# asharakeh/pod_compare

Measured on AMD Instinct MI355X. Metric: images/sec (BayesOD+MC-dropout, 1280x720), higher is better.
Workload: dtype f32 (convolutions: every fp32 product from 2-way f16 splits of the power-of-two-scaled fp32 operands, 3 partial products, fp32 accumulate; closer to fp64 than the fp32 MFMA: profiles/r05_f16_split_numerics.txt)

## Files before the change

### pod_compare_amd/csrc/k12_wino_conv_split.hip

```cpp
#include "pod_wino.h"

namespace pod {

typedef uint32_t vu32x4 __attribute__((ext_vector_type(4)));
constexpr int WINO_US_BYTES = 24 * 2 * 2 * 64 * 16;
constexpr int WINO_U_TOP = 14, WINO_V_TOP = 9;
constexpr int WINO_WAIT_VM24 = 0x4078;
constexpr int WINO_TAIL_NO_LOAD = 1, WINO_TAIL_NO_PARK = 2, WINO_TAIL_LAST = 4;

__global__ void __launch_bounds__(256) k_wino_filter_amax(const float* __restrict__ w, float* __restrict__ amax, int32_t K, int32_t C, int32_t Kpad) {
    const int64_t t = (int64_t)blockIdx.x * blockDim.x + threadIdx.x;
    float m = 0.0f;
    if (t < (int64_t)Kpad * C) {
        float u[4][6];
        wino_filter_values(w, (int)(t / C), (int)(t % C), K, C, u);
#pragma unroll
        for (int i = 0; i < 24; ++i) m = fmaxf(m, fabsf(u[i / 6][i % 6]));
    }
    wino_publish_amax1(amax, m);
}
__global__ void __launch_bounds__(256) k_wino_filter_split(const float* __restrict__ w, uint16_t* __restrict__ Us, const float* __restrict__ amax,
                                                           int32_t K, int32_t C, int32_t Kpad) {
    const int64_t t = (int64_t)blockIdx.x * blockDim.x + threadIdx.x;
    if (t >= (int64_t)Kpad * C) return;
    const int k = (int)(t / C), c = (int)(t % C);
    float u[4][6];
    wino_filter_values(w, k, c, K, C, u);
    const float sc = wino_pow2_scale(*amax, WINO_U_TOP);
    const int nchunk = C / 16, ks = k >> 6, kb = (k >> 5) & 1, j32 = k & 31, ch = c >> 4, hh = (c >> 3) & 1, e = c & 7;
    uint16_t* dst = Us + (((int64_t)ks * nchunk + ch) * (int64_t)WINO_US_BYTES) / 2 + (hh * 32 + j32) * 8 + e;
#pragma unroll
    for (int a = 0; a < 4; ++a)
#pragma unroll
        for (int p = 0; p < 6; ++p) {
            const float x = u[a][p] * sc;
            const _Float16 h0 = (_Float16)x;
            const _Float16 h1 = (_Float16)(x - (float)h0);
            uint16_t* d = dst + (((a * 6 + p) * 2 + kb) * 2) * 512;
            d[0] = __builtin_bit_cast(uint16_t, h0);
            d[512] = __builtin_bit_cast(uint16_t, h1);
        }
}

__global__ void __launch_bounds__(256, 1) k_wino_conv3x3_split(const WinoParams P) {
    extern __shared__ __attribute__((aligned(16))) float lds[];
    const int tid = threadIdx.x, lane = tid & 63, wave = tid >> 6;
    int ks, tb;
    wino_schedule(P.KS, P.n_blocks, ks, tb);
    if (tb >= P.n_blocks) return;
    uint32_t need[2] = {~0u, ~0u};
    if (P.live) {
        if (tb >= P.live[0]) return;
        const int32_t* const ent = P.live + POD_SPARSE_LIVE_HEAD + (int64_t)POD_SPARSE_LIVE_STRIDE * tb;
        tb = ent[0];
        need[0] = (uint32_t)ent[1 + (tid >> 5)];
        need[1] = (uint32_t)ent[9 + (tid >> 5 < 3 ? tid >> 5 : 2)];
    }
    WINO_STAMP(0);
    WINO_STAMP_WALL(12);
    uint32_t slot_e[12];
    int mini_pidx[3], dmini[3], doff[12];
    WINO_FILL_SLOTS(slot_e, mini_pidx, tid);
    const int nchunk_all = P.C >> 4;
    const int nchunk = P.c_split ? P.c_split : nchunk_all;
    const int chunk0 = (int)blockIdx.y * nchunk;
    const int i32 = lane & 31, h = lane >> 5;
    const int a = __builtin_amdgcn_readfirstlane(wave);
    const int set = (tb >= P.sets.first[1] ? 1 : 0) + (tb >= P.sets.first[2] ? 1 : 0) + (tb >= P.sets.first[3] ? 1 : 0);
    const float* const set_U = P.sets.U[set];
    const float* const set_in = P.sets.in[set];
    float* const set_out = P.sets.out[set];
    const float* const set_bias = P.sets.bias[set];
    const float in_amax_slot = wino_load_amax(P.sets.in_amax[set]);
    const float u_amax = *reinterpret_cast<const float*>(reinterpret_cast<const char*>(set_U) + (int64_t)P.KS * (P.C >> 4) * WINO_US_BYTES);
    float* const set_out_amax = P.sets.out_amax[set];
    const uint64_t set_offset = P.sets.offset[set];
    const int set_replicas = P.sets.replicas[set], set_k_planes = P.sets.k_planes[set];
    const auto u_rsrc = __builtin_amdgcn_make_buffer_rsrc(const_cast<char*>(reinterpret_cast<const char*>(set_U) + ((int64_t)ks * nchunk_all + chunk0) * WINO_US_BYTES), 0,
                                                          nchunk * WINO_US_BYTES, 0x00020000);
    const int u_off = (a * 6 * 4 * 64 + h * 32 + i32) * 16;
    constexpr int WINO_U_LEAD = 3;
    vu32x4 uP[6][4];
    auto filter_piece = [&](int q16, int p, vu32x4(&u)[4], int i) {
        u[i] = __builtin_bit_cast(vu32x4, __builtin_amdgcn_raw_buffer_load_b128(u_rsrc, u_off, q16 * WINO_US_BYTES + (p * 4 + i) * 1024, 0));
    };
#pragma unroll
    for (int pp = 0; pp < WINO_U_LEAD; ++pp)
#pragma unroll
        for (int i = 0; i < 4; ++i) filter_piece(0, pp, uP[pp], i);
    const WinoBlock B = wino_block(P.blocks[tb]);
    int row0, row1;
    float sgn;
    wino_rows(a, row0, row1, sgn);
    const int ty = i32 >> 2, tx = i32 & 3;
    const uint32_t lds_base = (uint32_t)(uintptr_t)(__attribute__((address_space(3))) float*)lds;
    uint32_t areg[2][2][2][2];
    uint32_t amini[2];
#pragma unroll
    for (int rs = 0; rs < 2; ++rs) {
        const int py = 2 * ty + (rs ? row1 : row0);
        const int p0 = 2 * (((py & 3) + 4 * (py >> 3)) * 18 + 4 * tx) + ((py >> 2) & 1);
#pragma unroll
        for (int cl = 0; cl < 2; ++cl) {
            const int rot = ((tx + cl) & 3) + 4 * ((py >> 1) & 1);
#pragma unroll
            for (int c16 = 0; c16 < 2; ++c16)
#pragma unroll
                for (int hf = 0; hf < 2; ++hf) areg[rs][cl][c16][hf] = lds_base + p0 * 128 + ((4 * c16 + 2 * h + hf + rot) & 7) * 16;
        }
    }
#pragma unroll
    for (int rs = 0; rs < 2; ++rs) amini[rs] = lds_base + 2 * WINO_SB_FLOATS * 4 + h * 12288 + ((2 * ty + (rs ? row1 : row0)) * 21 + tx) * 32;
    const auto r_rsrc = __builtin_amdgcn_make_buffer_rsrc(const_cast<float*>(set_in + B.base_px * P.in_stride + chunk0 * 16), 0,
                                                          B.n_img * B.HWi * P.in_stride * 4 - chunk0 * 64, 0x00020000);
    int* const pix_tab = wino_pixel_table(lds);
    WINO_FILL_PIXEL_TABLE(pix_tab, B, need, tid);
    wino_mini_offsets(&P, pix_tab, mini_pidx, dmini, lane);
    auto main_offsets = [&]() {
#pragma unroll
        for (int i = 0; i < 12; ++i) doff[i] = pix_tab[slot_e[i] & 0xFFFF];
#pragma unroll
        for (int i = 0; i < 12; ++i) doff[i] = wino_byte_offset(&P, doff[i], 4 * (((lane & 7) - (int)(slot_e[i] >> 16)) & 7));
    };

    f32x4 stg[6];
    const uint32_t stg_addr = lds_base + a * 12288 + lane * 16;
    auto stage_load = [&](int k, int sc, int i) {
        stg[k] = __builtin_bit_cast(f32x4, __builtin_amdgcn_raw_buffer_load_b128(r_rsrc, doff[i], sc * 128, 0));
    };
    auto stage_write = [&](int par, int k, int i) {
        *reinterpret_cast<__attribute__((address_space(3))) f32x4*>((uintptr_t)(stg_addr + par * (WINO_SB_FLOATS * 4) + i * 1024)) = stg[k];
    };

    f32x16 acc[12];
    f32x4 x[12];
    vu32x4 Vb[6][2];
    float tN[6][4], vN[2][6][4];
    if (POD_WINO_ELIM) {
#pragma unroll
    for (int i = 0; i < 12; ++i) Vb[i / 2][i % 2] = vu32x4{0x3c003c00u + i, 0x3c003c00u, 0x3c003c00u, 0x3c003c00u + lane};
#pragma unroll
    for (int i = 0; i < 12; ++i) x[i] = f32x4{1e-3f, 2e-3f, 3e-3f, 4e-3f} * (float)(lane + i);
#pragma unroll
    for (int i = 0; i < 48; ++i) vN[i / 24][(i / 4) % 6][i % 4] = x[i / 4][i % 4];
#pragma unroll
    for (int i = 0; i < 24; ++i) tN[i / 4][i % 4] = x[i / 4][i % 4];
    }
#define WINO_READ(par, c16, hf, i)                                                                                                  \
    asm volatile("ds_read_b128 %0, %1 offset:%2" : "=v"(x[i]) : "v"(areg[(i) / 6][((i) % 6) >> 2][c16][hf]), "i"((par) * WINO_SB_FLOATS * 4 + ((i) % 6) * 256))
#define WINO_READ_MINI(hf, i)                                                                                                        \
    asm volatile("ds_read_b128 %0, %1 offset:%2" : "=v"(x[i]) : "v"(amini[(i) / 6]), "i"((hf) * 16 + ((((i) % 6) & 3) * 5 + (((i) % 6) >> 2)) * 32))
#define WINO_READ12(M, ...)                                                                                                          \
    M(__VA_ARGS__, 0); M(__VA_ARGS__, 1); M(__VA_ARGS__, 2); M(__VA_ARGS__, 3); M(__VA_ARGS__, 4); M(__VA_ARGS__, 5);                \
    M(__VA_ARGS__, 6); M(__VA_ARGS__, 7); M(__VA_ARGS__, 8); M(__VA_ARGS__, 9); M(__VA_ARGS__, 10); M(__VA_ARGS__, 11)
#define WINO_READS_LANDED()                                                                                                           \
    asm volatile("s_waitcnt lgkmcnt(0)" : "+v"(x[0]), "+v"(x[1]), "+v"(x[2]), "+v"(x[3]), "+v"(x[4]), "+v"(x[5]), "+v"(x[6]), "+v"(x[7]), \
                 "+v"(x[8]), "+v"(x[9]), "+v"(x[10]), "+v"(x[11]))
    auto rows_combine = [&](int c0, int c1) __attribute__((always_inline)) {
#pragma unroll
        for (int c = c0; c < c1; ++c) {
#pragma unroll
            for (int e = 0; e < 4; ++e) tN[c][e] = __builtin_fmaf(sgn, x[6 + c][e], x[c][e]);
        }
    };
    float w0s[4], w1s[4], evs[4], ods[4], fs[4], gs[4];
    auto columns_level1 = [&](int e) __attribute__((always_inline)) {
        w0s[e] = __builtin_fmaf(-5.0f, tN[2][e], tN[4][e]);
        w1s[e] = __builtin_fmaf(-5.0f, tN[3][e], tN[5][e]);
        evs[e] = __builtin_fmaf(-4.0f, tN[2][e], tN[4][e]);
        ods[e] = __builtin_fmaf(-4.0f, tN[1][e], tN[3][e]);
        fs[e] = tN[4][e] - tN[2][e];
        gs[e] = tN[3][e] - tN[1][e];
    };
    auto columns_level2 = [&](int hf, int e) __attribute__((always_inline)) {
        vN[hf][0][e] = __builtin_fmaf(4.0f, tN[0][e], w0s[e]);
        vN[hf][5][e] = __builtin_fmaf(4.0f, tN[1][e], w1s[e]);
        vN[hf][1][e] = evs[e] + ods[e];
        vN[hf][2][e] = evs[e] - ods[e];
        vN[hf][3][e] = __builtin_fmaf(2.0f, gs[e], fs[e]);
        vN[hf][4][e] = __builtin_fmaf(-2.0f, gs[e], fs[e]);
    };
    const float sv = __builtin_bit_cast(float, __builtin_amdgcn_readfirstlane(__builtin_bit_cast(int, wino_pow2_scale(wino_reduce_amax(in_amax_slot), WINO_V_TOP))));
    auto split_convert = [&](int p, int term) __attribute__((always_inline)) {
        vu32x4 w;
#pragma unroll
        for (int i = 0; i < 4; ++i) {
            w[i] = term == 0 ? wino_f16_pair_scaled(vN[i >> 1][p][2 * (i & 1)], vN[i >> 1][p][2 * (i & 1) + 1], sv)
                             : wino_f16_pair(vN[i >> 1][p][2 * (i & 1)], vN[i >> 1][p][2 * (i & 1) + 1]);
        }
        Vb[p][term] = w;
    };
    auto split_residual = [&](int p, int i0, int i1) __attribute__((always_inline)) {
#pragma unroll
        for (int i = i0; i < i1; ++i) {
            float& lo = vN[i >> 1][p][2 * (i & 1)];
            float& hi = vN[i >> 1][p][2 * (i & 1) + 1];
            wino_f16_residual_scaled(Vb[p][0][i], lo, hi, sv);
        }
    };
    auto split_position = [&](int p) __attribute__((always_inline)) {
        split_convert(p, 0); split_residual(p, 0, 4); split_convert(p, 1);
    };
    auto make_v = [&](int hf) __attribute__((always_inline)) {
        if (POD_WINO_ELIM & 8) return;
        rows_combine(0, 6);
#pragma unroll
        for (int e = 0; e < 4; ++e) columns_level1(e);
#pragma unroll
        for (int e = 0; e < 4; ++e) columns_level2(hf, e);
    };
    auto split_all = [&]() __attribute__((always_inline)) {
        if (POD_WINO_ELIM & 8) return;
#pragma unroll
        for (int p = 0; p < 6; ++p) split_position(p);
    };

    constexpr int N_UNITS = 58, N_SLOTS = 36;
    auto unit = [&](auto U, auto npar_t, auto n16_t, auto hasA_t) __attribute__((always_inline)) {
        constexpr int u = decltype(U)::value, npar = decltype(npar_t)::value, n16 = decltype(n16_t)::value;
        if constexpr (POD_WINO_ELIM & 8) { if constexpr (u >= 3 && !(u >= 13 && u < 16)) return; }
        if constexpr (u < 3) {
            if constexpr (!(POD_WINO_ELIM & 1)) { WINO_READ(npar, n16, 0, 4 * u); WINO_READ(npar, n16, 0, 4 * u + 1); WINO_READ(npar, n16, 0, 4 * u + 2); WINO_READ(npar, n16, 0, 4 * u + 3); }
        } else if constexpr (u < 7) {
            if constexpr (decltype(hasA_t)::value) {
                constexpr int k = u - 3;
                if constexpr (k == 0) split_convert(5, 0);
                else if constexpr (k == 1) split_residual(5, 0, 2);
                else if constexpr (k == 2) split_residual(5, 2, 4);
                else split_convert(5, 1);
            }
        } else if constexpr (u < 13) {
            if constexpr (u == 7) WINO_READS_LANDED();
            rows_combine(u - 7, u - 6);
        } else if constexpr (u < 16) {
            if constexpr (!(POD_WINO_ELIM & 1)) { WINO_READ(npar, n16, 1, 4 * (u - 13)); WINO_READ(npar, n16, 1, 4 * (u - 13) + 1); WINO_READ(npar, n16, 1, 4 * (u - 13) + 2); WINO_READ(npar, n16, 1, 4 * (u - 13) + 3); }
        } else if constexpr (u < 24) {
            constexpr int k = u - 16;
            if constexpr (k < 4) columns_level1(k);
            else columns_level2(0, k - 4);
        } else if constexpr (u < 30) {
            if constexpr (u == 24) WINO_READS_LANDED();
            rows_combine(u - 24, u - 23);
        } else if constexpr (u < 38) {
            constexpr int k = u - 30;
            if constexpr (k < 4) columns_level1(k);
            else columns_level2(1, k - 4);
        } else {
            constexpr int p = (u - 38) / 4, k = (u - 38) % 4;
            if constexpr (k == 0) split_convert(p, 0);
            else if constexpr (k == 1) split_residual(p, 0, 2);
            else if constexpr (k == 2) split_residual(p, 2, 4);
            else split_convert(p, 1);
        }
    };
    const int last = nchunk - 1, last_s = last >> 1;
    const int sc1 = last_s < 1 ? last_s : 1;
#pragma unroll
    for (int r = 0; r < 3; ++r) wino_mini_piece(r_rsrc, lds, a, 0, r, dmini[r]);
#pragma unroll
    for (int r = 0; r < 3; ++r) wino_mini_piece(r_rsrc, lds, a, 1, r, dmini[r]);
    WINO_STAMP(9);
    main_offsets();
    WINO_STAMP(10);
#pragma unroll
    for (int i = 0; i < 12; ++i) wino_patch_piece(r_rsrc, lds, a, 0, i, doff[i]);
#pragma unroll
    for (int i = 0; i < 6; ++i) wino_patch_piece(r_rsrc, lds + WINO_SB_FLOATS, a, sc1, i, doff[i]);
#pragma unroll
    for (int i = 0; i < 6; ++i) stage_load(i, sc1, 6 + i);
    WINO_STAMP(11);
    __builtin_amdgcn_s_waitcnt(WINO_WAIT_VM24);
    __builtin_amdgcn_s_barrier();
    WINO_STAMP(1);
    WINO_READ12(WINO_READ_MINI, 0);
    WINO_READS_LANDED();
    __builtin_amdgcn_sched_barrier(0);
    make_v(0);
    __builtin_amdgcn_sched_barrier(0);
    WINO_READ12(WINO_READ_MINI, 1);
    WINO_READS_LANDED();
    __builtin_amdgcn_sched_barrier(0);
    make_v(1);
    split_all();
    __builtin_amdgcn_sched_barrier(0);
    WINO_STAMP(2);
    const f32x16 zero16 = {0.f, 0.f, 0.f, 0.f, 0.f, 0.f, 0.f, 0.f, 0.f, 0.f, 0.f, 0.f, 0.f, 0.f, 0.f, 0.f};
    auto chunk = [&](auto mode_t, auto c16_t, auto par_t, auto tail_t, int q) {
        constexpr int mode = decltype(mode_t)::value, c16 = decltype(c16_t)::value, par = decltype(par_t)::value, tail = decltype(tail_t)::value;
        constexpr bool do_load = !(tail & WINO_TAIL_NO_LOAD), do_park = !(tail & WINO_TAIL_NO_PARK), is_last = (tail & WINO_TAIL_LAST) != 0;
        static_assert((tail == 0 || mode == 2) && (!is_last || (!do_load && !do_park)), "tail forms are steady-state chunks; the last one has no stage traffic");
        constexpr int n16 = c16 ^ 1, npar = c16 == 1 ? par ^ 1 : par;
        const int qn = q + 1 <= last ? q + 1 : last;
        const int ls0 = (q >> 1) + 2, ls = ls0 < last_s ? ls0 : last_s;
        wino_static_for([&](auto J) __attribute__((always_inline)) {
            constexpr int j = decltype(J)::value, p = j / 6, m = j % 6, kb = m & 1, prod = m >> 1;
            constexpr int sa = prod == 1 ? 1 : 0;
            constexpr int sb = prod == 0 ? 1 : 0;
            if constexpr (mode == 0 && prod == 0)
                acc[p * 2 + kb] = __builtin_amdgcn_mfma_f32_32x32x16_f16(__builtin_bit_cast(wino_f16x8, uP[p][kb * 2 + sa]), __builtin_bit_cast(wino_f16x8, Vb[p][sb]), zero16, 0, 0, 0);
            else
                acc[p * 2 + kb] = __builtin_amdgcn_mfma_f32_32x32x16_f16(__builtin_bit_cast(wino_f16x8, uP[p][kb * 2 + sa]), __builtin_bit_cast(wino_f16x8, Vb[p][sb]), acc[p * 2 + kb], 0, 0, 0);
            if constexpr (m < 4 && (!is_last || p + WINO_U_LEAD < 6)) { if (!(POD_WINO_ELIM & 2)) filter_piece(p + WINO_U_LEAD >= 6 ? qn : q, (p + WINO_U_LEAD) % 6, uP[(p + WINO_U_LEAD) % 6], m); }
            if constexpr (m == 4 && do_park) { if (!(POD_WINO_ELIM & 4)) stage_write(c16 == 0 ? par ^ 1 : par, p, c16 == 0 ? 6 + p : p); }
            if constexpr (p == 5 && m >= 4 && do_load) {
                if (!(POD_WINO_ELIM & 4)) {
                    stage_load(3 * (m - 4), ls, 6 * c16 + 3 * (m - 4));
                    stage_load(3 * (m - 4) + 1, ls, 6 * c16 + 3 * (m - 4) + 1);
                    stage_load(3 * (m - 4) + 2, ls, 6 * c16 + 3 * (m - 4) + 2);
                }
            }
            if constexpr (mode != 0) {
                constexpr int u0 = j * N_UNITS / N_SLOTS, u1 = (j + 1) * N_UNITS / N_SLOTS;
                wino_static_for([&](auto K) __attribute__((always_inline)) {
                    constexpr int u = u0 + decltype(K)::value;
                    if constexpr (!is_last || (u >= 3 && u < 7))
                        unit(std::integral_constant<int, u>{}, std::integral_constant<int, npar>{}, std::integral_constant<int, n16>{}, std::integral_constant<bool, mode == 2>{});
                }, std::make_integer_sequence<int, u1 - u0>{});
            }
            __builtin_amdgcn_sched_barrier(0);
        }, std::make_integer_sequence<int, N_SLOTS>{});
        if constexpr (do_park) {
            __builtin_amdgcn_s_waitcnt(WINO_WAIT_LGKM0);
            __builtin_amdgcn_s_barrier();
        }
        if constexpr (mode == 0) {
            if (q >= last) return;
            if constexpr (!(POD_WINO_ELIM & 1)) WINO_READ12(WINO_READ, npar, n16, 0);
            WINO_READS_LANDED();
            __builtin_amdgcn_sched_barrier(0);
            make_v(0);
            __builtin_amdgcn_sched_barrier(0);
            if constexpr (!(POD_WINO_ELIM & 1)) WINO_READ12(WINO_READ, npar, n16, 1);
            WINO_READS_LANDED();
            __builtin_amdgcn_sched_barrier(0);
            make_v(1);
            split_all();
            __builtin_amdgcn_sched_barrier(0);
            __builtin_amdgcn_s_barrier();
        }
    };
    using std::integral_constant;
    constexpr integral_constant<int, 0> I0{};
    constexpr integral_constant<int, 1> I1{};
    constexpr integral_constant<int, 2> I2{};
    const bool peel = (nchunk & 3) == 0;
    const int nloop = peel ? nchunk - 4 : nchunk;
    chunk(I0, I0, I0, I0, 0);
    if (nchunk > 1) chunk(I1, I1, I0, I0, 1);
    for (int base = 0;; base += 4) {
#define WINO_CHUNK(t)                                                                                                              \
    if (base + (t) >= nloop) break;                                                                                                \
    chunk(I2, integral_constant<int, (t) & 1>{}, integral_constant<int, ((t) >> 1) & 1>{}, I0, base + (t));
        WINO_CHUNK(2) WINO_CHUNK(3) WINO_CHUNK(4) WINO_CHUNK(5)
#undef WINO_CHUNK
    }
    if (peel) {
        if (nchunk > 4) {
            chunk(I2, I0, I0, integral_constant<int, WINO_TAIL_NO_LOAD>{}, nchunk - 4);
            chunk(I2, I1, I0, integral_constant<int, WINO_TAIL_NO_LOAD | WINO_TAIL_NO_PARK>{}, nchunk - 3);
        }
        chunk(I2, I0, I1, integral_constant<int, WINO_TAIL_NO_LOAD | WINO_TAIL_NO_PARK>{}, nchunk - 2);
        chunk(I2, I1, I1, integral_constant<int, WINO_TAIL_NO_LOAD | WINO_TAIL_NO_PARK | WINO_TAIL_LAST>{}, nchunk - 1);
    }
    __syncthreads();
    WINO_STAMP(3);

    if (!wino_output_stage(acc, lds, a, i32, h)) return;
    const float inv = wino_pow2_inverse(sv) * wino_pow2_inverse(wino_pow2_scale(u_amax, WINO_U_TOP));
    const WinoStore S{set_out + (int64_t)blockIdx.y * P.split_out_stride, set_bias, set_out_amax, inv, set_offset, set_replicas, set_k_planes};
    const float lmax = S.k_planes > 0 ? wino_store_planes(P, B, S, lds, ks) : wino_store_channels_last(P, B, S, lds, ks);
    if (set_out_amax) wino_publish_amax_block(set_out_amax, lmax);
    WINO_STAMP_END();
}

}

#ifdef POD_TRACE
extern "C" int pod_wino_trace_dump_split(long long* host, int32_t n_workgroups) { return pod::wino_trace_dump(host, n_workgroups); }
#endif

extern "C" int64_t pod_wino_filter_split_bytes(int32_t K, int32_t C) {
    if (K < 1 || C < 16 || (C & 15) != 0) return 0;
    const int64_t Kpad = (K + 63) / 64 * 64;
    return Kpad / 64 * (C / 16) * (int64_t)pod::WINO_US_BYTES + 16;
}

extern "C" int pod_wino_filter_transform_split(const float* weight, void* Us, int32_t K, int32_t C, pod_stream_t stream) {
    if (!weight || !Us || K < 1 || C < 16 || (C & 15) != 0 || !pod_aligned(16, Us)) return POD_E_INVALID;
    const int32_t Kpad = (K + 63) / 64 * 64;
    const int64_t n = (int64_t)Kpad * C;
    float* amax = reinterpret_cast<float*>(reinterpret_cast<char*>(Us) + pod_wino_filter_split_bytes(K, C) - 16);
    if (hipMemsetAsync(amax, 0, 16, (hipStream_t)stream) != hipSuccess) return POD_E_LAUNCH;
    hipLaunchKernelGGL(pod::k_wino_filter_amax, dim3((unsigned)((n + 255) / 256)), dim3(256), 0, (hipStream_t)stream, weight, amax, K, C, Kpad);
    POD_CHECK_LAUNCH();
    hipLaunchKernelGGL(pod::k_wino_filter_split, dim3((unsigned)((n + 255) / 256)), dim3(256), 0, (hipStream_t)stream, weight,
                       reinterpret_cast<uint16_t*>(Us), amax, K, C, Kpad);
    POD_CHECK_LAUNCH();
    return POD_OK;
}

extern "C" int pod_wino_conv3x3_split(const PodWinoConv* d, pod_stream_t stream) {
    if (!d || d->n_sets < 1 || d->n_sets > 4 || !d->blocks || d->n_blocks < 0 || d->C < 16 || (d->C & 15) != 0 || d->K < 64 || (d->K & 63) != 0 ||
        !(d->p >= 0.0f && d->p < 1.0f) || d->sets[0].first_block != 0 || !pod_aligned(16, d->blocks) ||
        d->reserved != 0)
        return POD_E_INVALID;
    const int32_t C = d->C, K = d->K;
    pod::WinoParams P{};
    const int64_t grid = pod::wino_params_launch(P, d->blocks, d->n_blocks, C, K, d->relu, d->p, d->seed, d->epoch);
    if (grid < 0) return POD_E_INVALID;
    const bool partial = d->n_splits > 1;
    if (partial) {
        if (d->n_sets != 1 || d->n_splits > 16 || (C / 16) % d->n_splits != 0 || ((C / 16 / d->n_splits) & 1) != 0 || d->split_stride < 0 || (d->split_stride & 3) != 0 ||
            d->p != 0.0f || d->relu || d->sets[0].bias || d->sets[0].replicas || d->sets[0].k_planes || d->sets[0].out_amax)
            return POD_E_INVALID;
    }
    for (int s = 0; s < 4; ++s) {
        const PodConvSet& q = d->sets[s < d->n_sets ? s : 0];
        if (s < d->n_sets) {
            if (!q.in || !q.out || q.in == q.out || !q.Us || !q.in_amax || q.replicas < 0 || q.replicas > 127 || q.k_planes < 0 || q.k_planes > K ||
                (q.k_planes > 0 && (d->p != 0.0f || q.replicas != 0)) || (s > 0 && q.first_block < d->sets[s - 1].first_block) || q.first_block > d->n_blocks)
                return POD_E_INVALID;
            if (!pod_aligned(16, q.in, q.out, q.Us, q.bias) || !pod_aligned(4, q.in_amax, q.out_amax))
                return POD_E_INVALID;
        }
        pod::wino_params_set(P, s, s < d->n_sets ? q.first_block : INT32_MAX, q.in, q.out, q.Us, q.bias, q.in_amax, q.out_amax, q.offset, q.replicas, q.k_planes);
    }
    if (d->n_blocks == 0) return POD_OK;
    if (pod_lds_opt_in<pod::k_wino_conv3x3_split>(pod::WINO_LDS_BYTES) != POD_OK) return POD_E_LAUNCH;
    P.c_split = partial ? C / 16 / d->n_splits : 0; P.split_out_stride = partial ? d->split_stride : 0;
    P.live = d->live_blocks;
    hipLaunchKernelGGL(pod::k_wino_conv3x3_split, dim3((unsigned)grid, partial ? (unsigned)d->n_splits : 1u), dim3(256), pod::WINO_LDS_BYTES, (hipStream_t)stream, P);
    POD_CHECK_LAUNCH();
    return POD_OK;
}
```

### pod_compare_amd/csrc/pod_wino.h

```cpp
#pragma once
#include "pod_experiments.h"
#include "pod_split_gemm.h"

namespace pod {

constexpr int WINO_U_FLOATS = 24 * 2 * 64 * 4;
constexpr int WINO_SB_FLOATS = 384 * 32;
constexpr int WINO_LDS_BYTES = 4 * 32 * 4 * 65 * 4;

#ifdef POD_TRACE
static __device__ long long g_wino_trace[8192 * 16];
#define WINO_STAMP(k)                                                                                          \
    do {                                                                                                       \
        if (threadIdx.x == 0 && blockIdx.x < 8192) g_wino_trace[blockIdx.x * 16 + (k)] = __builtin_readcyclecounter(); \
    } while (0)
#define WINO_STAMP_WALL(k)                                                                                     \
    do {                                                                                                       \
        if (threadIdx.x == 0 && blockIdx.x < 8192) g_wino_trace[blockIdx.x * 16 + (k)] = wall_clock64();       \
    } while (0)
#define WINO_STAMP_END()                                                                                       \
    do {                                                                                                       \
        __builtin_amdgcn_s_waitcnt(0);                                                                         \
        WINO_STAMP(5);                                                                                         \
        WINO_STAMP_WALL(13);                                                                                   \
        if (threadIdx.x == 0 && blockIdx.x < 8192) {                                                           \
            uint32_t hw, xcc;                                                                                  \
            asm volatile("s_getreg_b32 %0, hwreg(HW_REG_HW_ID)" : "=s"(hw));                                   \
            asm volatile("s_getreg_b32 %0, hwreg(HW_REG_XCC_ID)" : "=s"(xcc));                                 \
            g_wino_trace[blockIdx.x * 16 + 6] = ((long long)xcc << 32) | hw;                                   \
        }                                                                                                      \
    } while (0)
static inline int wino_trace_dump(long long* host, int32_t n_workgroups) {
    if (hipDeviceSynchronize() != hipSuccess) return POD_E_LAUNCH;
    if (n_workgroups > 8192) n_workgroups = 8192;
    if (hipMemcpyFromSymbol(host, HIP_SYMBOL(g_wino_trace), (size_t)n_workgroups * 16 * sizeof(long long)) != hipSuccess) return POD_E_LAUNCH;
    return POD_OK;
}
#else
#define WINO_STAMP(k)
#define WINO_STAMP_WALL(k)
#define WINO_STAMP_END()
#endif

constexpr int WINO_WAIT_VM4 = 0x0074, WINO_WAIT_VM0 = 0x0070, WINO_WAIT_VM16 = 0x4070, WINO_WAIT_LGKM0 = 0xC07F;

struct WinoParams {
    const int4* blocks;
    int32_t n_blocks, C, K, KS, in_stride, out_stride, relu;
    uint32_t thresh;
    float scale;
    uint64_t seed;
    int32_t c_split;
    int64_t split_out_stride;
    const uint64_t* epoch;
    const int32_t* live;
    struct Sets {
        int32_t first[4];
        const float* in[4];
        float* out[4];
        const float* U[4];
        const float* bias[4];
        const float* in_amax[4];
        float* out_amax[4];
        uint64_t offset[4];
        int32_t replicas[4];
        int32_t k_planes[4];
    } sets;
};

struct WinoSlotTable {
    uint32_t v[384];
    constexpr WinoSlotTable() : v() {
        for (int p = 0; p < 384; ++p) {
            const int cls = p & 1, k = p >> 1, rr = k / 18, px = k - rr * 18;
            const int py = cls ? (rr < 4 ? rr + 4 : rr + 8) : (rr < 4 ? rr : rr < 8 ? rr + 4 : rr + 8);
            const bool ok = cls ? rr < 8 : rr < 10;
            v[p] = ok ? (uint32_t)((py * 18 + px) | ((((px >> 2) & 3) + 4 * ((py >> 1) & 1)) << 16)) : 324u;
        }
    }
};
static __device__ const WinoSlotTable g_wino_slots{};

__device__ __forceinline__ void wino_schedule(int KS, int n_blocks, int& ks, int& tb) {
    const int xcd = blockIdx.x & 7, wi = (int)(blockIdx.x >> 3);
    const int SP = KS >= 2 ? 2 : 1, G = KS / SP;
    ks = SP * (xcd % G) + (wi % SP);
    tb = (wi / SP) * (8 / G) + xcd / G;
}
inline int64_t wino_grid(int KS, int64_t n_blocks) {
    const int SP = KS >= 2 ? 2 : 1, G = KS / SP;
    return 8 * SP * ((n_blocks * G + 7) / 8);
}
inline int64_t wino_params_launch(WinoParams& P, const int32_t* blocks, int32_t n_blocks, int32_t C, int32_t K, int32_t relu, float p, uint64_t seed,
                                  const uint64_t* epoch) {
    const int32_t KS = K / 64;
    if (KS != 1 && KS != 2 && KS != 4 && KS != 8) return -1;
    P.blocks = reinterpret_cast<const int4*>(blocks);
    P.n_blocks = n_blocks; P.C = C; P.K = K; P.KS = KS; P.in_stride = C; P.out_stride = K; P.relu = relu;
    P.thresh = POD_DROPOUT_THRESH16(p);
    P.scale = 1.0f / (1.0f - p);
    P.seed = seed; P.epoch = epoch;
    const int64_t grid = wino_grid(KS, n_blocks);
    return grid > 0x7FFFFFFFLL ? -1 : grid;
}
inline void wino_params_set(WinoParams& P, int s, int32_t first, const float* in, float* out, const void* U, const float* bias, const float* in_amax,
                            float* out_amax, uint64_t offset, int32_t replicas, int32_t k_planes) {
    P.sets.first[s] = first;
    P.sets.in[s] = in; P.sets.out[s] = out; P.sets.U[s] = reinterpret_cast<const float*>(U); P.sets.bias[s] = bias;
    P.sets.in_amax[s] = in_amax; P.sets.out_amax[s] = out_amax;
    P.sets.offset[s] = offset; P.sets.replicas[s] = replicas; P.sets.k_planes[s] = k_planes;
}

template <typename T>
__device__ __forceinline__ void wino_pin_one(T& v) {
    asm volatile("" : "+v"(v));
}
template <typename... T>
__device__ __forceinline__ void wino_pin(T&... v) {
    (wino_pin_one(v), ...);
}

__device__ __forceinline__ void wino_filter_values(const float* __restrict__ w, int k, int c, int K, int C, float (&u)[4][6]) {
    float g[3][3];
#pragma unroll
    for (int i = 0; i < 9; ++i) g[i / 3][i % 3] = k < K ? w[((int64_t)k * C + c) * 9 + i] : 0.0f;
    float t0[4][3];
#pragma unroll
    for (int j = 0; j < 3; ++j) {
        t0[0][j] = g[0][j];
        t0[1][j] = 0.5f * (g[0][j] + g[1][j] + g[2][j]);
        t0[2][j] = 0.5f * (g[0][j] - g[1][j] + g[2][j]);
        t0[3][j] = g[2][j];
    }
#pragma unroll
    for (int a = 0; a < 4; ++a) {
        const float x0 = t0[a][0], x1 = t0[a][1], x2 = t0[a][2];
        u[a][0] = 0.25f * x0;
        u[a][1] = (-1.0f / 6.0f) * (x0 + x1 + x2);
        u[a][2] = (-1.0f / 6.0f) * (x0 - x1 + x2);
        u[a][3] = (1.0f / 24.0f) * x0 + (1.0f / 12.0f) * x1 + (1.0f / 6.0f) * x2;
        u[a][4] = (1.0f / 24.0f) * x0 - (1.0f / 12.0f) * x1 + (1.0f / 6.0f) * x2;
        u[a][5] = x2;
    }
}

struct WinoBlock {
    int64_t base_px, out_px;
    int gcols, H, W, n_img, y0, x0, Hv, Wv, HWi;
    float rHv, rWv;
};
__device__ __forceinline__ WinoBlock wino_block(const int4 desc) {
    WinoBlock B;
    B.base_px = desc.x; B.out_px = desc.y;
    B.gcols = (desc.z >> 24) & 0xFF; B.H = (desc.z >> 12) & 0xFFF; B.W = desc.z & 0xFFF; B.n_img = (desc.w >> 24) & 0xFF;
    B.y0 = ((desc.w >> 12) & 0xFFF) * 16; B.x0 = (desc.w & 0xFFF) * 16; B.Wv = B.W + 1; B.Hv = B.H + 1; B.HWi = B.H * B.W;
    B.rWv = 1.0f / (float)B.Wv; B.rHv = 1.0f / (float)B.Hv;
    return B;
}
__device__ __forceinline__ int wino_cell(int v, int step, float rstep, int& idx) {
    int n = (int)((float)v * rstep);
    n -= n * step > v ? 1 : 0;
    n += (n + 1) * step <= v ? 1 : 0;
    idx = n;
    return v - n * step;
}

__device__ __forceinline__ void wino_rows(int a, int& row0, int& row1, float& sgn) {
    row0 = a == 0 ? 0 : a == 2 ? 2 : 1;
    row1 = a == 2 ? 1 : a == 3 ? 3 : 2;
    sgn = a == 1 ? 1.0f : -1.0f;
}

__device__ __forceinline__ int* wino_pixel_table(float* lds) { return reinterpret_cast<int*>(lds + 2 * WINO_SB_FLOATS + 2 * 3072); }
#define WINO_FILL_PIXEL_TABLE(pix_tab, B, need, tid)                                                                                  \
    _Pragma("unroll") for (int it_ = 0; it_ < 2; ++it_) {                                                                             \
        const int t = (tid) + 256 * it_;                                                                                              \
        if (t >= 325) break;                                                                                                          \
        const int py = t / 18, px = t - py * 18, vy = (B).y0 - 1 + py, vx = (B).x0 - 1 + px;                                          \
        int m, n;                                                                                                                     \
        const int gy = wino_cell(vy < 0 ? 0 : vy, (B).Hv, (B).rHv, m), gx = wino_cell(vx < 0 ? 0 : vx, (B).Wv, (B).rWv, n), img = m * (B).gcols + n; \
        const bool ok = (t < 324) & (vy >= 0) & (gy < (B).H) & (vx >= 0) & (gx < (B).W) & (n < (B).gcols) & (img < (B).n_img) & ((((need)[it_] >> (t & 31)) & 1u) != 0); \
        (pix_tab)[t] = ok ? img * (B).HWi + gy * (B).W + gx : -1;       \
    }                                                                                                                                 \
    __syncthreads();                                                                                                                  \
    WINO_STAMP(8)

#define WINO_FILL_SLOTS(slot_e, mini_pidx, tid)                                                                                       \
    _Pragma("unroll") for (int i = 0; i < 12; ++i) (slot_e)[i] = g_wino_slots.v[96 * ((tid) >> 6) + 8 * i + (((tid) & 63) >> 3)];     \
    _Pragma("unroll") for (int r = 0; r < 3; ++r) {                                                                                   \
        const int pp = ((((tid) >> 6) * 3 + r) * 64 + ((tid) & 63)) >> 1, py = pp / 21, pi = pp - py * 21, px = 4 * (pi % 5) + pi / 5; \
        (mini_pidx)[r] = py < 18 && pi < 20 && px < 18 ? py * 18 + px : 324;                                                          \
    }
__device__ __forceinline__ int wino_byte_offset(const WinoParams* P, int pix, int part4) {
    return pix >= 0 ? (pix * P->in_stride + part4) * 4 : 0x7FFFFF00;
}
__device__ __forceinline__ void wino_mini_offsets(const WinoParams* P, const int* pix_tab, const int (&mini_pidx)[3], int (&dmini)[3], int lane) {
#pragma unroll
    for (int r = 0; r < 3; ++r) dmini[r] = pix_tab[mini_pidx[r]];
#pragma unroll
    for (int r = 0; r < 3; ++r) dmini[r] = wino_byte_offset(P, dmini[r], 4 * (lane & 1));
}
typedef __attribute__((address_space(3))) void wino_lds_void;
__device__ __forceinline__ void wino_mini_piece(__amdgpu_buffer_rsrc_t rsrc, float* lds, int a, int which, int r, int dmini_r) {
    __builtin_amdgcn_raw_ptr_buffer_load_lds(rsrc, (wino_lds_void*)(lds + 2 * WINO_SB_FLOATS + which * 3072 + (a * 3 + r) * 256), 16, dmini_r, which * 32, 0, 0);
}
__device__ __forceinline__ void wino_patch_piece(__amdgpu_buffer_rsrc_t rsrc, float* stage, int a, int sc, int i, int doff_i) {
    __builtin_amdgcn_raw_ptr_buffer_load_lds(rsrc, (wino_lds_void*)(stage + (a * 12 + i) * 256), 16, doff_i, sc * 128, 0, 0);
}

constexpr int WINO_TS = 260;
constexpr int WINO_ZA = 32 * WINO_TS;
__device__ __forceinline__ bool wino_output_stage(const f32x16 (&acc)[12], float* lds, int a, int i32, int h) {
    if (POD_WINO_ELIM & 128) {
#pragma unroll
        for (int i = 0; i < 12; ++i) asm volatile("" ::"v"(acc[i]));
        return false;
    }
#pragma unroll
    for (int kb = 0; kb < 2; ++kb)
#pragma unroll
        for (int g = 0; g < 4; ++g) {
            f32x4 m[6];
#pragma unroll
            for (int p6 = 0; p6 < 6; ++p6) m[p6] = f32x4{acc[p6 * 2 + kb][4 * g], acc[p6 * 2 + kb][4 * g + 1], acc[p6 * 2 + kb][4 * g + 2], acc[p6 * 2 + kb][4 * g + 3]};
            const f32x4 s1 = m[1] + m[2], d1 = m[1] - m[2], s2 = m[3] + m[4], d2 = m[3] - m[4];
            float* o = lds + (a * 32 + i32) * WINO_TS + kb * 32 + 8 * g + 4 * h;
            *reinterpret_cast<f32x4*>(o) = (m[0] + s1) + s2;
            *reinterpret_cast<f32x4*>(o + 64) = __builtin_elementwise_fma(f32x4{2.f, 2.f, 2.f, 2.f}, d2, d1);
            *reinterpret_cast<f32x4*>(o + 128) = __builtin_elementwise_fma(f32x4{4.f, 4.f, 4.f, 4.f}, s2, s1);
            *reinterpret_cast<f32x4*>(o + 192) = __builtin_elementwise_fma(f32x4{8.f, 8.f, 8.f, 8.f}, d2, d1) + m[5];
        }
    __syncthreads();
    WINO_STAMP(4);
    return !(POD_WINO_ELIM & 32);
}

struct WinoStore {
    float* out;
    const float* bias;
    float* out_amax;
    float inv;
    uint64_t offset;
    int replicas, k_planes;
};
__device__ __forceinline__ void wino_dropout8(f32x4& v0, f32x4& v1, int64_t e, uint64_t offset, uint32_t word, uint64_t key, uint32_t thresh, float scale) {
    const uint64_t ctr = offset + (uint64_t)(e >> 3);
    const u32x4 r4 = philox4x32_10(u32x4{(uint32_t)ctr, (uint32_t)(ctr >> 32), word, STREAM_DROPOUT}, (uint32_t)key, (uint32_t)(key >> 32));
    dropout_mask4(v0, r4.x, r4.y, thresh, scale);
    dropout_mask4(v1, r4.z, r4.w, thresh, scale);
}


template <bool RELU, bool AMAX>
__device__ __forceinline__ float wino_store_planes_form(const WinoBlock& B, const WinoStore& S, const float* lds, int ks) {
    const int tid = threadIdx.x, wave = __builtin_amdgcn_readfirstlane(tid >> 6);
    float lmax = 0.0f;
    const f32x4 inv = f32x4{S.inv, S.inv, S.inv, S.inv};
    const int oy = (tid >> 2) & 15, ox = (tid & 3) * 4, odd = oy & 1;
    const float sg = odd ? -1.0f : 1.0f;
    const int kg0 = ks * 64 + wave;
    const int n_it = (S.k_planes - kg0 + 3) >> 2;
    const float bias_l = S.bias ? S.bias[kg0 + 4 * (tid & 15)] : 0.0f;
    int m;
    const int gy = wino_cell(B.y0 + oy, B.Hv, B.rHv, m);
    int64_t px0[4];
#pragma unroll
    for (int e = 0; e < 4; ++e) {
        int n;
        const int gx = wino_cell(B.x0 + ox + e, B.Wv, B.rWv, n), img = m * B.gcols + n;
        px0[e] = (n < B.gcols && img < B.n_img && gx < B.W && gy < B.H) ? (B.out_px + (int64_t)img * B.HWi) * S.k_planes + (int64_t)gy * B.W + gx : -1;
    }
    const bool vec = px0[0] >= 0 && px0[3] == px0[0] + 3 && (px0[0] & 3) == 0 && (B.HWi & 3) == 0;
    const bool ok[4] = {px0[0] >= 0, px0[1] >= 0, px0[2] >= 0, px0[3] >= 0};
    int64_t q[4];
#pragma unroll
    for (int e = 0; e < 4; ++e) q[e] = (int64_t)kg0 * B.HWi + px0[e];
    const int64_t q_it = (int64_t)4 * B.HWi;
    const int tile = (oy >> 1) * 4 + (tid & 3);
    const float* r = lds + tile * WINO_TS + wave + (odd ? WINO_ZA : 0);
#pragma unroll 1
    for (int it0 = 0; it0 < 16 && it0 < n_it; it0 += 4, r += 16) {
        float z[4][4][3];
        f32x4 v[4];
#pragma unroll
        for (int j = 0; j < 4; ++j)
#pragma unroll
            for (int e = 0; e < 4; ++e)
#pragma unroll
                for (int a = 0; a < 3; ++a) z[j][e][a] = r[4 * j + e * 64 + a * WINO_ZA];
#pragma unroll
        for (int j = 0; j < 4; ++j) {
            const float bias = __builtin_bit_cast(float, __builtin_amdgcn_readlane(__builtin_bit_cast(int, bias_l), it0 + j));
            f32x4 y;
#pragma unroll
            for (int e = 0; e < 4; ++e) y[e] = __builtin_fmaf(sg, z[j][e][2], __builtin_fmaf(sg, z[j][e][1], z[j][e][0]));
            v[j] = __builtin_elementwise_fma(y, inv, f32x4{bias, bias, bias, bias});
            if (RELU) wino_relu4(v[j]);
            if (AMAX) {
                const float mx = wino_absmax4(0.0f, f32x4{ok[0] ? v[j].x : 0.f, ok[1] ? v[j].y : 0.f, ok[2] ? v[j].z : 0.f, ok[3] ? v[j].w : 0.f});
                lmax = fmaxf(lmax, it0 + j < n_it ? mx : 0.0f);
            }
        }
        wino_pin(v[0], v[1], v[2], v[3]);
#pragma unroll
        for (int j = 0; j < 4; ++j) {
            const bool live = it0 + j < n_it;
            if (live && vec) {
                *reinterpret_cast<f32x4*>(S.out + q[0]) = v[j];
            } else if (live) {
                if (ok[0]) S.out[q[0]] = v[j].x;
                if (ok[1]) S.out[q[1]] = v[j].y;
                if (ok[2]) S.out[q[2]] = v[j].z;
                if (ok[3]) S.out[q[3]] = v[j].w;
            }
#pragma unroll
            for (int e = 0; e < 4; ++e) q[e] += q_it;
        }
    }
    return lmax;
}
__device__ __forceinline__ float wino_store_planes(const WinoParams& P, const WinoBlock& B, const WinoStore& S, const float* lds, int ks) {
    switch ((P.relu ? 1 : 0) | (S.out_amax ? 2 : 0)) {
        case 0: return wino_store_planes_form<false, false>(B, S, lds, ks);
        case 1: return wino_store_planes_form<true, false>(B, S, lds, ks);
        case 2: return wino_store_planes_form<false, true>(B, S, lds, ks);
        default: return wino_store_planes_form<true, true>(B, S, lds, ks);
    }
}

template <bool RELU, bool DROP>
__device__ __forceinline__ float wino_store_channels_last_form(const WinoParams& P, const WinoBlock& B, const WinoStore& S, const float* lds, int ks) {
    const int tid = threadIdx.x;
    float lmax = 0.0f;
    const f32x4 inv = f32x4{S.inv, S.inv, S.inv, S.inv};
    const int k8 = (tid & 7) * 8, kg = ks * 64 + k8, ox = (tid >> 3) & 15, odd = tid >> 7;
    const float sg1 = odd ? -1.0f : 1.0f;
    const f32x4 sg = f32x4{sg1, sg1, sg1, sg1};
    f32x4 bias0 = f32x4{0.f, 0.f, 0.f, 0.f}, bias1 = bias0;
    if (S.bias) {
        bias0 = *reinterpret_cast<const f32x4*>(S.bias + kg);
        bias1 = *reinterpret_cast<const f32x4*>(S.bias + kg + 4);
    }
    const uint64_t drop_key = DROP ? dropout_key(P.seed, P.epoch) : 0ull;
    const int n_rep = S.replicas > 0 ? S.replicas : 1;
    const uint32_t word = S.replicas > 0 ? 2u : 0u;
    int n, m;
    const int gx = wino_cell(B.x0 + ox, B.Wv, B.rWv, n);
    const bool col_ok = n < B.gcols && gx < B.W;
    int gy = wino_cell(B.y0 + odd, B.Hv, B.rHv, m);
    int img = m * B.gcols + n;
    const int64_t e_row = (int64_t)(2 * B.W) * P.out_stride, e_wrap = ((int64_t)B.gcols * B.HWi - (int64_t)B.Hv * B.W) * P.out_stride, e_rep = (int64_t)B.HWi * P.out_stride;
    int64_t e = (B.out_px + (int64_t)img * B.HWi + (int64_t)gy * B.W + gx) * P.out_stride + kg - e_row;
    gy -= 2;
    const float* rbase = lds + (ox >> 2) * WINO_TS + (ox & 3) * 64 + k8 + (odd ? WINO_ZA : 0);
#pragma unroll 1
    for (int g = 0; g < 2; ++g) {
        f32x4 z[4][6], v[4][2];
        bool ok[4];
        int64_t er[4];
#pragma unroll
        for (int it = 0; it < 4; ++it) {
            gy += 2;
            const bool wrap = gy >= B.Hv;
            gy -= wrap ? B.Hv : 0;
            img += wrap ? B.gcols : 0;
            e += e_row + (wrap ? e_wrap : 0);
            ok[it] = col_ok && gy < B.H && img < B.n_img;
            er[it] = e;
            const float* r = rbase + (4 * g + it) * 4 * WINO_TS;
            z[it][0] = *reinterpret_cast<const f32x4*>(r); z[it][1] = *reinterpret_cast<const f32x4*>(r + 4);
            z[it][2] = *reinterpret_cast<const f32x4*>(r + WINO_ZA); z[it][3] = *reinterpret_cast<const f32x4*>(r + WINO_ZA + 4);
            z[it][4] = *reinterpret_cast<const f32x4*>(r + 2 * WINO_ZA); z[it][5] = *reinterpret_cast<const f32x4*>(r + 2 * WINO_ZA + 4);
        }
#pragma unroll
        for (int it = 0; it < 4; ++it) {
            v[it][0] = __builtin_elementwise_fma(__builtin_elementwise_fma(sg, z[it][4], __builtin_elementwise_fma(sg, z[it][2], z[it][0])), inv, bias0);
            v[it][1] = __builtin_elementwise_fma(__builtin_elementwise_fma(sg, z[it][5], __builtin_elementwise_fma(sg, z[it][3], z[it][1])), inv, bias1);
            if (RELU) {
                wino_relu4(v[it][0]);
                wino_relu4(v[it][1]);
            }
            const float mx = wino_absmax4(wino_absmax4(0.0f, v[it][0]), v[it][1]);
            lmax = fmaxf(lmax, ok[it] ? (DROP ? mx * P.scale : mx) : 0.0f);
        }
#pragma unroll 1
        for (int rep = 0; rep < n_rep; ++rep) {
            f32x4 w[4][2];
#pragma unroll
            for (int it = 0; it < 4; ++it) {
                w[it][0] = v[it][0];
                w[it][1] = v[it][1];
                if (DROP && !(POD_WINO_ELIM & 64)) wino_dropout8(w[it][0], w[it][1], er[it], S.offset, word, drop_key, P.thresh, P.scale);
            }
#pragma unroll
            for (int it = 0; it < 4; ++it) wino_pin(w[it][0], w[it][1]);
#pragma unroll
            for (int it = 0; it < 4; ++it) {
                if (ok[it]) {
                    *reinterpret_cast<f32x4*>(S.out + er[it]) = w[it][0];
                    *reinterpret_cast<f32x4*>(S.out + er[it] + 4) = w[it][1];
                }
                er[it] += e_rep;
            }
        }
    }
    return lmax;
}
__device__ __forceinline__ float wino_store_channels_last(const WinoParams& P, const WinoBlock& B, const WinoStore& S, const float* lds, int ks) {
    switch ((P.relu ? 1 : 0) | (P.thresh ? 2 : 0)) {
        case 0: return wino_store_channels_last_form<false, false>(P, B, S, lds, ks);
        case 1: return wino_store_channels_last_form<true, false>(P, B, S, lds, ks);
        case 2: return wino_store_channels_last_form<false, true>(P, B, S, lds, ks);
        default: return wino_store_channels_last_form<true, true>(P, B, S, lds, ks);
    }
}

}
```

Baseline: 145.4.

## Pre-scale Winograd input tiles at LDS park time instead of during f16 split

Moves the power-of-two input scale from the per-element f16 split and residual steps to the point where input pixels are parked into LDS. Raw buffer loads go to registers, are multiplied by the scale, then written to LDS. The prologue loads that went directly to LDS now go through registers and are parked later, interleaved into the first MFMA iteration. This removes the scaled conversion variants from the hot transform path, but raises VGPR pressure through the 18+6 held f32x4 registers and adds VALU multiplies on the park path.

```diff
diff --git a/pod_compare_amd/csrc/k12_wino_conv_split.hip b/pod_compare_amd/csrc/k12_wino_conv_split.hip
--- a/pod_compare_amd/csrc/k12_wino_conv_split.hip
+++ b/pod_compare_amd/csrc/k12_wino_conv_split.hip
@@ -124,12 +124,13 @@
     };
 
     f32x4 stg[6];
-    const uint32_t stg_addr = lds_base + a * 12288 + lane * 16;
+    const uint32_t stg_addr = wino_stage_park_base(lds_base, a, lane);
+    float sv;
     auto stage_load = [&](int k, int sc, int i) {
         stg[k] = __builtin_bit_cast(f32x4, __builtin_amdgcn_raw_buffer_load_b128(r_rsrc, doff[i], sc * 128, 0));
     };
     auto stage_write = [&](int par, int k, int i) {
-        *reinterpret_cast<__attribute__((address_space(3))) f32x4*>((uintptr_t)(stg_addr + par * (WINO_SB_FLOATS * 4) + i * 1024)) = stg[k];
+        wino_park_scaled(stg_addr + par * (WINO_SB_FLOATS * 4) + i * 1024, stg[k], sv);
     };
 
     f32x16 acc[12];
@@ -180,13 +181,11 @@
         vN[hf][3][e] = __builtin_fmaf(2.0f, gs[e], fs[e]);
         vN[hf][4][e] = __builtin_fmaf(-2.0f, gs[e], fs[e]);
     };
-    const float sv = __builtin_bit_cast(float, __builtin_amdgcn_readfirstlane(__builtin_bit_cast(int, wino_pow2_scale(wino_reduce_amax(in_amax_slot), WINO_V_TOP))));
     auto split_convert = [&](int p, int term) __attribute__((always_inline)) {
         vu32x4 w;
 #pragma unroll
         for (int i = 0; i < 4; ++i) {
-            w[i] = term == 0 ? wino_f16_pair_scaled(vN[i >> 1][p][2 * (i & 1)], vN[i >> 1][p][2 * (i & 1) + 1], sv)
-                             : wino_f16_pair(vN[i >> 1][p][2 * (i & 1)], vN[i >> 1][p][2 * (i & 1) + 1]);
+            w[i] = wino_f16_pair(vN[i >> 1][p][2 * (i & 1)], vN[i >> 1][p][2 * (i & 1) + 1]);
         }
         Vb[p][term] = w;
     };
@@ -195,7 +194,7 @@
         for (int i = i0; i < i1; ++i) {
             float& lo = vN[i >> 1][p][2 * (i & 1)];
             float& hi = vN[i >> 1][p][2 * (i & 1) + 1];
-            wino_f16_residual_scaled(Vb[p][0][i], lo, hi, sv);
+            wino_f16_residual(Vb[p][0][i], lo, hi);
         }
     };
     auto split_position = [&](int p) __attribute__((always_inline)) {
@@ -255,21 +254,27 @@
     };
     const int last = nchunk - 1, last_s = last >> 1;
     const int sc1 = last_s < 1 ? last_s : 1;
-#pragma unroll
-    for (int r = 0; r < 3; ++r) wino_mini_piece(r_rsrc, lds, a, 0, r, dmini[r]);
-#pragma unroll
-    for (int r = 0; r < 3; ++r) wino_mini_piece(r_rsrc, lds, a, 1, r, dmini[r]);
+    f32x4 mini[6], pre[18];
+#pragma unroll
+    for (int r = 0; r < 3; ++r) mini[r] = wino_mini_piece_load(r_rsrc, 0, dmini[r]);
+#pragma unroll
+    for (int r = 0; r < 3; ++r) mini[3 + r] = wino_mini_piece_load(r_rsrc, 1, dmini[r]);
     WINO_STAMP(9);
+    sv = __builtin_bit_cast(float, __builtin_amdgcn_readfirstlane(__builtin_bit_cast(int, wino_pow2_scale(wino_reduce_amax(in_amax_slot), WINO_V_TOP))));
     main_offsets();
     WINO_STAMP(10);
 #pragma unroll
-    for (int i = 0; i < 12; ++i) wino_patch_piece(r_rsrc, lds, a, 0, i, doff[i]);
-#pragma unroll
-    for (int i = 0; i < 6; ++i) wino_patch_piece(r_rsrc, lds + WINO_SB_FLOATS, a, sc1, i, doff[i]);
+    for (int i = 0; i < 12; ++i) pre[i] = wino_patch_piece_load(r_rsrc, 0, doff[i]);
+#pragma unroll
+    for (int i = 0; i < 6; ++i) pre[12 + i] = wino_patch_piece_load(r_rsrc, sc1, doff[i]);
 #pragma unroll
     for (int i = 0; i < 6; ++i) stage_load(i, sc1, 6 + i);
     WINO_STAMP(11);
     __builtin_amdgcn_s_waitcnt(WINO_WAIT_VM24);
+    const uint32_t mini_addr = wino_mini_park_base(lds_base, a, lane);
+#pragma unroll
+    for (int r = 0; r < 6; ++r) wino_park_scaled(mini_addr + (r / 3) * 12288 + (r % 3) * 1024, mini[r], sv);
+    __builtin_amdgcn_s_waitcnt(WINO_WAIT_LGKM0);
     __builtin_amdgcn_s_barrier();
     WINO_STAMP(1);
     WINO_READ12(WINO_READ_MINI, 0);
@@ -302,6 +307,10 @@
                 acc[p * 2 + kb] = __builtin_amdgcn_mfma_f32_32x32x16_f16(__builtin_bit_cast(wino_f16x8, uP[p][kb * 2 + sa]), __builtin_bit_cast(wino_f16x8, Vb[p][sb]), acc[p * 2 + kb], 0, 0, 0);
             if constexpr (m < 4 && (!is_last || p + WINO_U_LEAD < 6)) { if (!(POD_WINO_ELIM & 2)) filter_piece(p + WINO_U_LEAD >= 6 ? qn : q, (p + WINO_U_LEAD) % 6, uP[(p + WINO_U_LEAD) % 6], m); }
             if constexpr (m == 4 && do_park) { if (!(POD_WINO_ELIM & 4)) stage_write(c16 == 0 ? par ^ 1 : par, p, c16 == 0 ? 6 + p : p); }
+            if constexpr (mode == 0 && p >= 2 && m != 4 && (p - 2) * 5 + (m < 4 ? m : 4) < 18) {
+                constexpr int n = (p - 2) * 5 + (m < 4 ? m : 4);
+                wino_park_scaled(stg_addr + (n < 12 ? n * 1024 : WINO_SB_FLOATS * 4 + (n - 12) * 1024), pre[n], sv);
+            }
             if constexpr (p == 5 && m >= 4 && do_load) {
                 if (!(POD_WINO_ELIM & 4)) {
                     stage_load(3 * (m - 4), ls, 6 * c16 + 3 * (m - 4));
diff --git a/pod_compare_amd/csrc/pod_wino.h b/pod_compare_amd/csrc/pod_wino.h
--- a/pod_compare_amd/csrc/pod_wino.h
+++ b/pod_compare_amd/csrc/pod_wino.h
@@ -207,6 +207,26 @@
 __device__ __forceinline__ void wino_patch_piece(__amdgpu_buffer_rsrc_t rsrc, float* stage, int a, int sc, int i, int doff_i) {
     __builtin_amdgcn_raw_ptr_buffer_load_lds(rsrc, (wino_lds_void*)(stage + (a * 12 + i) * 256), 16, doff_i, sc * 128, 0, 0);
 }
+__device__ __forceinline__ f32x4 wino_mini_piece_load(__amdgpu_buffer_rsrc_t rsrc, int which, int dmini_r) {
+    return __builtin_bit_cast(f32x4, __builtin_amdgcn_raw_buffer_load_b128(rsrc, dmini_r, which * 32, 0));
+}
+__device__ __forceinline__ f32x4 wino_patch_piece_load(__amdgpu_buffer_rsrc_t rsrc, int sc, int doff_i) {
+    return __builtin_bit_cast(f32x4, __builtin_amdgcn_raw_buffer_load_b128(rsrc, doff_i, sc * 128, 0));
+}
+__device__ __forceinline__ uint32_t wino_mini_park_base(uint32_t lds_base, int a, int lane) { return lds_base + 2 * WINO_SB_FLOATS * 4 + a * 3072 + lane * 16; }
+__device__ __forceinline__ uint32_t wino_stage_park_base(uint32_t lds_base, int a, int lane) { return lds_base + a * 12288 + lane * 16; }
+__device__ __forceinline__ void wino_park_scaled(uint32_t lds_byte, const f32x4& v, float s) {
+    f32x4 w;
+    asm("v_mul_f32 %0, %1, %2" : "=v"(w.x) : "s"(s), "v"(v.x));
+    asm("v_mul_f32 %0, %1, %2" : "=v"(w.y) : "s"(s), "v"(v.y));
+    asm("v_mul_f32 %0, %1, %2" : "=v"(w.z) : "s"(s), "v"(v.z));
+    asm("v_mul_f32 %0, %1, %2" : "=v"(w.w) : "s"(s), "v"(v.w));
+    *reinterpret_cast<__attribute__((address_space(3))) f32x4*>((uintptr_t)lds_byte) = w;
+}
+__device__ __forceinline__ void wino_f16_residual(uint32_t w, float& lo, float& hi) {
+    asm("v_fma_mix_f32 %0, %0, 1.0, -%1 op_sel_hi:[0,0,1]" : "+v"(lo) : "v"(w));
+    asm("v_fma_mix_f32 %0, %0, 1.0, -%1 op_sel:[0,0,1] op_sel_hi:[0,0,1]" : "+v"(hi) : "v"(w));
+}
 
 constexpr int WINO_TS = 260;
 constexpr int WINO_ZA = 32 * WINO_TS;
```

New measurement: 146.0, median of 6. Within noise of the previous version (+0.4%).
